# vfrantc/Bayesian-Enhancement-Model

Hardware: AMD Instinct MI355X
Metric: images/sec (whole node) CG_UNet N=8 Bayesian eval @256x256 (higher is better)
Workload: dtype f32

## Files before the change

bayesian-enhancement-model_amd/bem/native.py:

```python
from __future__ import annotations

import ctypes
import os
from ctypes import c_double, c_float, c_int, c_int64, c_uint64, c_void_p

_HERE = os.path.dirname(os.path.abspath(__file__))
LIB_PATH = os.environ.get("BEM_HIP_LIB", os.path.join(os.path.dirname(_HERE), "lib", "libbem_hip.so"))
CSRC = os.path.join(os.path.dirname(_HERE), "csrc")


class BemNativeError(RuntimeError):
    pass


class PwArgs(ctypes.Structure):
    _fields_ = [
        ("x1", c_void_p), ("x2", c_void_p), ("C1", c_int), ("C2", c_int), ("in_mode", c_int),
        ("ln_w", c_void_p), ("ln_b", c_void_p), ("ln_eps", c_float),
        ("Wp", c_void_p), ("w_bstride", c_int64),
        ("bias", c_void_p), ("bias_bstride", c_int64),
        ("res", c_void_p),
        ("prelu", c_void_p), ("act", c_int),
        ("out", c_void_p), ("out_mode", c_int), ("Win", c_int),
        ("B", c_int), ("M", c_int), ("K", c_int), ("L", c_int),
# ... 29 lines not shown
    "bem_pack_pw_weight_f32": [P, P, I, I, I, P],
    "bem_pw_packed_elems": [I, I],
    "bem_pw_gemm_x6_f32": [ctypes.POINTER(PwArgs), P],
    "bem_pack_pw_weight_x6": [P, P, I, I, I, P],
    "bem_pack_pw_weight_x6_strided": [P, P, I, I, I, I64, I64, I64, P],
    "bem_pack_pw_weight_x6_jobs": [P, P, I, P, P],
    "bem_pw_x6_packed_elems": [I, I],
    "bem_bnn_sample_pack_x6": [P, P, P, P, I, I, I, U64, U64, P, I, P],
    "bem_store_words": [P, P, I, P],
    "bem_bnn_ebank_sample_f32": [P, P, I, P, U64, U64, P],
    "bem_bnn_bank_sample_f32": [P, P, I, P, P, P, P, P, F, P, U64, U64, P, P],
    "bem_bnn_bank_kl_f32": [P, P, I, P, P, P, P],
    "bem_bnn_bank_kl_bwd_f32": [P, P, I, P, P, P, P],
    "bem_bnn_bank_reparam_bwd_f32": [P, P, I, P, P, P],
    "bem_row_scale_f32": [P, P, P, I, I, P],
    "bem_se_gate_f32": [P, P, P, P, I, I, I, P],
    "bem_spatial_attention_f32": [P, P, P, P, P, I, I, I, I, I, P],
    "bem_hamilton_bwd_f32": [P, P, P, I, I, I, P],
    "bem_chan_scale_f32": [P, P, I64, P, P, F, P, I, I, I64, P],
    "bem_chan_dot_f32": [P, P, P, I, I, I64, I, P],
    "bem_se_gate_bwd_f32": [P, P, P, P, P, P, P, P, I, I, I, P],
    "bem_spatial_attention_bwd_f32": [P, P, P, P, P, P, P, I, I, I, I, I, P],
    "bem_bnn_prior_ema_f32": [P, P, P, P, F, P, I64, P],
    "bem_bnn_kl_f32": [P, P, P, P, I64, P, P],
    "bem_bnn_kl_bwd_f32": [P, P, P, P, I64, P, P, P, P],
    "bem_bnn_reparam_bwd_f32": [P, P, P, P, P, I64, P],
    "bem_mask_token_f32": [P, P, P, P, I, I, I, I, P],
    "bem_mask_token_bwd_f32": [P, P, P, P, I, I, I, I, P],
    "bem_depth_to_space_f32": [P, P, I, I, I, I, P],
    "bem_prelu_f32": [P, P, P, I64, P],
    "bem_prelu_bwd_f32": [P, P, P, P, P, I64, P],
    "bem_bilinear_up_bwd_f32": [P, P, I, I, I, I, I, P],
    "bem_gdmlp_x6_f32": [P, P, P, F, P, P, P, P, P, P, I, I, I, I, I, P],
    "bem_conv3x3_x6_f32": [P, I64, P, P, P, P, P, I, I, I, I, I, I, P],
    "bem_conv4x4s2_x6_f32": [P, I64, P, P, P, P, P, I, I, I, I, I, I, P],
    "bem_conv4x4s2_fast_supported": [I, I, I],
    "bem_conv3x3_rows_supported": [I, I, I],
    "bem_ss2d_front_x6_f32": [P, P, P, F, P, P, P, P, P, P, P, I, I, I, I, I, P],
    "bem_conv_taps_x6_f32": [P, I64, P, P, P, P, P, I, I, I, I, I, I, I, I, I, P],
    "bem_dwconv3x3_f32": [P, P, I64, P, I64, P, I, I, I, I, I, P],
    "bem_conv2d_f32": [P, I64, P, P, P, P, P, I, I, I, I, I, I, I, I, I, I, P],
    "bem_conv2d_mfma_f32": [P, I64, P, P, P, P, P, I, I, I, I, I, I, I, I, I, I, P],
    "bem_quat_dwt_f32": [P, I64, P, I, I, I, P],
    "bem_dwt_f32": [P, P, I, I, I, I, P],
    "bem_iwt_f32": [P, P, I, I, I, I, P],
    "bem_iwt_hamilton_f32": [P, P, P, I, I, I, P],
    "bem_hamilton_f32": [P, P, I, I, I, P],
    "bem_hamilton_full_f32": [P, P, P, I, I, I, P],
    "bem_attn_stats_f64": [P, P, P, I, I, P],
    "bem_attn_fold_f32": [P, P, P, P, P, P, I, I, P],
    "bem_transpose_planes_f32": [P, I64, P, I64, I, I, I, I, P],
    "bem_copy_channels_f32": [P, I64, P, I64, I, I, I, P],
    "bem_copy_channels_rep_f32": [P, I64, P, I64, I, I, I, I, P],
    "bem_add_channels_f32": [P, I64, P, I64, I, I, I, P],
    "bem_bilinear_up_f32": [P, I64, P, I64, I, I, I, I, I, P],
    "bem_space_to_depth_f32": [P, P, I, I, I, I, P],
    "bem_pixel_shuffle2_f32": [P, P, I, I, I, I, P],
    "bem_bnn_sample_f32": [P, P, P, P, I, I64, U64, U64, P, P],
    "bem_select_best_f32": [P, P, P, P, P, I, I, I64, P],
    "bem_ssim_f32": [P, P, P, P, I, I, I, I, P],
    "bem_select_scores_f32": [P, P, P, F, I, P, P, P, P, I, I, I64, P],
    "bem_mc_mean_f32": [P, P, P, P, I, I, I, I, I, I, I, P],
    "bem_pad_reflect_f32": [P, P, I, I, I, I, I, P],
    "bem_resize_down_f32": [P, P, I, I, I, I, P],
    "bem_randn_f32": [P, I64, U64, U64, P, P],
    "bem_cond_postproc_f32": [P, P, P, P, I, I, I, I, F, P],
# ... 57 lines not shown
```

bayesian-enhancement-model_amd/bem/ops.py:

```python
from __future__ import annotations

import ctypes
import os
from typing import Optional

import torch

from . import native
from .native import PwArgs, check, lib


def _stream():
    return ctypes.c_void_p(torch.cuda.current_stream().cuda_stream)


def _p(t: Optional[torch.Tensor]):
    return ctypes.c_void_p(0 if t is None else t.data_ptr())


def _chk(t: Optional[torch.Tensor], name: str, dtype=torch.float32, optional=False):
    if t is None:
        if optional:
            return
        raise ValueError(f"{name} is required")
# ... 246 lines not shown
    if ln_w.numel() != C or ln_b.numel() != C or dww.numel() != 9 * C or (dwb is not None and dwb.numel() != C) or (bias_in is not None and bias_in.numel() != C):
        raise ValueError("ss2d_front: parameter shapes")
    for Wp, (M, K), nm in ((Wp_in, (C, C), "Wp_in"), (Wp_x, (Mx, C), "Wp_x")):
        if Wp.dim() != 2 or Wp.shape[0] != 1 or Wp.shape[1] != packed_elems(M, K, True) or getattr(Wp, "_bem_mk", (M, K)) != (M, K):
            raise ValueError(f"ss2d_front: {nm} {tuple(Wp.shape)} does not match M={M} K={K} (x6 format, one weight set)")
    xc = torch.empty_like(x)
    xd = torch.empty(B, Mx, H, W, device=x.device, dtype=x.dtype)
    check(lib().bem_ss2d_front_x6_f32(_p(x), _p(ln_w), _p(ln_b), float(ln_eps), _p(Wp_in), _p(bias_in), _p(dww), _p(dwb), _p(Wp_x), _p(xc), _p(xd),
                                      B, C, Mx, H, W, _stream()), "ss2d_front")
    return xc, xd


def gate_interleave(Hd, device):
    j = torch.arange(Hd // 16, device=device)[:, None, None]
    c = torch.arange(16, device=device)[None, :, None]
    s_ = torch.arange(2, device=device)[None, None, :]
    return (s_ * Hd + 16 * j + c).reshape(-1)


GDMLP_X6 = os.environ.get("BEM_GDMLP_X6", "1") != "0"
GDMLP_X6_MAXC = int(os.environ.get("BEM_GDMLP_X6_MAXC", "80"))


def gdmlp_x6_supported(C, Hd):
    return USE_X6 and GDMLP_X6 and C <= GDMLP_X6_MAXC and Hd % 16 == 0


def dw_gate_params10(dww, dwb, Hd):
    w = dww.reshape(2, Hd, 9).permute(1, 2, 0)
    b = torch.zeros(Hd, 1, 2, device=dww.device, dtype=dww.dtype) if dwb is None else dwb.reshape(2, Hd).t().reshape(Hd, 1, 2)
    return torch.cat([w, b], 1).contiguous()


def gdmlp_x6(x, ln_w, ln_b, ln_eps, Wp_gate, bias_gate, dw10, Wp_out, bias_out, Hd):
    for n_, t in (("x", x), ("ln_w", ln_w), ("ln_b", ln_b), ("Wp_gate", Wp_gate), ("bias_gate", bias_gate), ("dw10", dw10), ("Wp_out", Wp_out)):
        _chk(t, n_)
    _chk(bias_out, "bias_out", optional=True)
    B, C, H, W = x.shape
    if not (USE_X6 and C <= 80 and Hd % 16 == 0):
        raise ValueError(f"gdmlp_x6: C = {C} (<= 80) / Hd = {Hd} (% 16) not supported")
    if tuple(dw10.shape) != (Hd, 10, 2):
        raise ValueError("gdmlp_x6: depthwise parameters must come from dw_gate_params10")
    if ln_w.numel() != C or ln_b.numel() != C or bias_gate.numel() != 2 * Hd or (bias_out is not None and bias_out.numel() != C):
        raise ValueError("gdmlp_x6: parameter shapes")
    for Wp, (M, K), nm in ((Wp_gate, (2 * Hd, C), "Wp_gate"), (Wp_out, (C, Hd), "Wp_out")):
        if Wp.dim() != 2 or Wp.shape[0] != 1 or Wp.shape[1] != packed_elems(M, K, True) or getattr(Wp, "_bem_mk", (M, K)) != (M, K):
            raise ValueError(f"gdmlp_x6: {nm} {tuple(Wp.shape)} does not match M={M} K={K} (x6 format, one weight set)")
    out = torch.empty_like(x)
    s = _timed("gdmlp_x6", 8.0 * x.numel(), 6.0 * 2.0 * B * H * W * (2 * Hd * C + Hd * C)) if _PROF is not None and _PROF["kernel"] == "gdmlp_x6" and _PROF["pred"](C) else None
    check(lib().bem_gdmlp_x6_f32(_p(x), _p(ln_w), _p(ln_b), float(ln_eps), _p(Wp_gate), _p(bias_gate), _p(dw10), _p(Wp_out),
                                 _p(bias_out), _p(out), B, C, Hd, H, W, _stream()), "gdmlp_x6")
    _timed_end(s)
    return out


def dwconv3x3(x, w, bias=None, mode=0):
    _chk(x, "x"); _chk(w, "w"); _chk(bias, "bias", optional=True)
    B, Cin, H, W = x.shape
    Cout = Cin // 2 if mode == 2 else Cin
    per_b = w.dim() == 5
    Cw = w.shape[1] if per_b else w.shape[0]
    if Cw != Cin or tuple(w.shape[-3:]) != (1, 3, 3) or (per_b and w.shape[0] != B):
        raise ValueError(f"dwconv3x3: weight {tuple(w.shape)} vs input channels {Cin}")
    bb = 0
    if bias is not None:
        if bias.shape[-1] != Cin:
# ... 961 lines not shown
```

bayesian-enhancement-model_amd/csrc/gdmlp_x6.hip:

```cpp
#include "bem_common.h"
#include "x6_common.h"

namespace {

struct GdX {
    const float* x; const float* ln_w; const float* ln_b; float ln_eps;
    const u32x4* Wpi;
    const u32x4* Wpo;
    const float* bgi;
    const float* dw10;
    int C, Hd, H, W, NCH, tx;
};

constexpr int GD_TH = 4, GD_TW = 32, GD_HW = GD_TW + 2;
constexpr int GD_NPH = (GD_TH + 2) * GD_HW;
constexpr int GD_NPB = (GD_NPH + 31) / 32;
constexpr int GD_TS = 208;
constexpr int GD_GS = 20;

typedef float f32x4 __attribute__((ext_vector_type(4)));

__device__ __forceinline__ float gelu_gate1(float a, float b) {
    const float t = __builtin_amdgcn_rcpf(fmaf(0.3275911f * 0.70710678118654752440f, fabsf(a), 1.f));
    float p = fmaf(1.061405429f, t, -1.453152027f);
    p = fmaf(p, t, 1.421413741f);
    p = fmaf(p, t, -0.284496736f);
    p = fmaf(p, t, 0.254829592f);
    const float e = __builtin_amdgcn_exp2f(a * a * -0.72134752044448170368f);
    const float r = fmaf(-(p * t), e, 1.f);
    const float h = 0.5f * a;
    return fmaf(h, copysignf(r, a), h) * b;
}

template <int KBM, int MTO, int WOB, bool PL2>
__global__ __launch_bounds__(256, 2) void gdmlp_x6_kernel(GdX k, const float* __restrict__ bpo, float bomul, float* __restrict__ out) {
    constexpr int NPI = 3 * KBM, NPO = 3 * MTO;
    __shared__ __attribute__((aligned(16))) f32x2 T[16 * GD_TS];
    __shared__ __attribute__((aligned(16))) float G[128 * GD_GS];
    __shared__ __attribute__((aligned(16))) u32x4 Wis[2][NPI * 64];
    __shared__ __attribute__((aligned(16))) u32x4 Wos[WOB][NPO * 64];
    __shared__ __attribute__((aligned(16))) f32x2 Bss[2][16];
    __shared__ __attribute__((aligned(16))) f32x2 DWs[2][16 * 10];
    const int lane = threadIdx.x & 63, wave = __builtin_amdgcn_readfirstlane(threadIdx.x >> 6), kh = lane >> 5, n = lane & 31;
    const int b = blockIdx.z;
    const int tile = xcd_tile(blockIdx.x, gridDim.x);
    const int tyi = tile / k.tx, txi = tile - tyi * k.tx;
    const int y0 = tyi * GD_TH, x0 = txi * GD_TW;
    const int L = k.H * k.W;
    const float* xb = k.x + (int64_t)b * k.C * L;

    const uint32_t voff = 16 * lane;
    const uint32_t wi_lds = lds_addr(Wis), wo_lds = lds_addr(Wos), bs_lds = lds_addr(Bss), dw_lds = lds_addr(DWs);
    auto dma_in = [&](int ji, int buf) {
#pragma unroll
        for (int t = 0; t < (NPI + 3) / 4; ++t) {
            const int p = wave + 4 * t;
            if (p < NPI) glds16(k.Wpi + ((int64_t)ji * NPI + p) * 64, voff, wi_lds + (buf * NPI + p) * 1024);
        }
        if (wave == (NPI & 3)) {
            const float* src = k.dw10 + (int64_t)ji * 320;
            glds16(src, voff, dw_lds + buf * 1280);
            if (lane < 16) glds16(src + 256, voff, dw_lds + buf * 1280 + 1024);
        }
        if (wave == ((NPI + 1) & 3) && lane < 8) glds16(k.bgi + (int64_t)ji * 32, voff, bs_lds + buf * 128);
    };
    auto dma_out = [&](int jo, int buf) {
#pragma unroll
        for (int t = 0; t < (NPO + 3) / 4; ++t) {
            const int p = wave + 4 * t, mt = p / 3, li = p - 3 * mt;
            if (p < NPO) glds16(k.Wpo + (((int64_t)mt * k.NCH + jo) * 3 + li) * 64, voff, wo_lds + (buf * NPO + p) * 1024);
        }
    };
    dma_in(0, 0);

    const int oy = y0 + wave, ox = x0 + n;
    f32x16 rs[MTO];
    const bool opix = oy < k.H && ox < k.W;
    const int64_t po = (int64_t)min(oy, k.H - 1) * k.W + min(ox, k.W - 1);
    auto load_res = [&]() {
        const float* rb = xb + po;
#pragma unroll
        for (int mt = 0; mt < MTO; ++mt)
#pragma unroll
            for (int r = 0; r < 16; ++r) {
                const int row = min(32 * mt + (r & 3) + 8 * (r >> 2) + 4 * kh, k.C - 1);
                rs[mt][r] = fmaf(bpo[row], bomul, rb[(int64_t)row * L]);
            }
    };

    u32x4 xl[2][KBM][3];
    float msk[2];
    uint32_t mbit[2];
    int hpo[2];
    {
        float lnw[KBM][8], lnb[KBM][8];
#pragma unroll
        for (int kb = 0; kb < KBM; ++kb)
#pragma unroll
            for (int e = 0; e < 8; ++e) {
                const int ch = 16 * kb + 8 * kh + e;
                const float on = ch < k.C ? 1.f : 0.f;
                lnw[kb][e] = k.ln_w[min(ch, k.C - 1)] * on;
                lnb[kb][e] = k.ln_b[min(ch, k.C - 1)] * on;
            }
        float xr[2][KBM][8];
        auto load_block = [&](int i) {
            const int hp = min((wave + 4 * i) * 32 + n, GD_TS - 1);
            hpo[i] = hp;
            const int hy = hp / GD_HW, hx = hp - hy * GD_HW;
            const int gy = y0 - 1 + hy, gx = x0 - 1 + hx;
            const bool in = hp < GD_NPH && gy >= 0 && gy < k.H && gx >= 0 && gx < k.W && (wave + 4 * i) < GD_NPB;
            msk[i] = in ? 1.f : 0.f;
            mbit[i] = in ? 0xffffffffu : 0u;
            const int off = min(max(gy, 0), k.H - 1) * k.W + min(max(gx, 0), k.W - 1);
#pragma unroll
            for (int kb = 0; kb < KBM; ++kb)
#pragma unroll
                for (int e = 0; e < 8; ++e) {
                    const int ch = 16 * kb + 8 * kh + e;
                    const float v = xb[(int64_t)min(ch, k.C - 1) * L + off];
                    xr[i][kb][e] = ch < k.C ? v : 0.f;
                }
        };
        auto norm_block = [&](int i) {
            const float inv = 1.f / (float)k.C;
            float s = 0.f;
#pragma unroll
            for (int kb = 0; kb < KBM; ++kb)
#pragma unroll
                for (int e = 0; e < 8; ++e) s += xr[i][kb][e];
            s += __shfl_xor(s, 32, 64);
            const float mean = s * inv;
            float q = 0.f;
#pragma unroll
            for (int kb = 0; kb < KBM; ++kb)
#pragma unroll
                for (int e = 0; e < 8; ++e) {
                    const float d = (16 * kb + 8 * kh + e < k.C) ? xr[i][kb][e] - mean : 0.f;
                    q = fmaf(d, d, q);
                }
            q += __shfl_xor(q, 32, 64);
            const float rstd = msk[i] / sqrtf(q * inv + k.ln_eps);
#pragma unroll
            for (int kb = 0; kb < KBM; ++kb) {
                float v[8];
#pragma unroll
                for (int e = 0; e < 8; ++e) v[e] = ((xr[i][kb][e] - mean) * rstd) * lnw[kb][e] + lnb[kb][e] * msk[i];
                split8(v, xl[i][kb][0], xl[i][kb][1], xl[i][kb][2]);
            }
        };
        if (PL2) { load_block(0); load_block(1); norm_block(0); norm_block(1); }
        else { load_block(0); norm_block(0); load_block(1); norm_block(1); }
    }

    const int wb_lds = 2 * kh * GD_HW + n;
    const int c_lo = 4 * wave;

    f32x16 oh[MTO];
#pragma unroll
    for (int mt = 0; mt < MTO; ++mt)
#pragma unroll
        for (int r = 0; r < 16; ++r) oh[mt][r] = 0.f;

    auto phase_c = [&](const u32x4* Wo) {
        const float* gp = G + (wave * 32 + n) * GD_GS + 8 * kh;
        const f32x4 ga = *reinterpret_cast<const f32x4*>(gp), gb = *reinterpret_cast<const f32x4*>(gp + 4);
        const float v[8] = {ga[0], ga[1], ga[2], ga[3], gb[0], gb[1], gb[2], gb[3]};
        u32x4 gl[3];
        split8(v, gl[0], gl[1], gl[2]);
#pragma unroll
        for (int mt = 0; mt < MTO; ++mt) {
            const u32x4* wp = Wo + mt * 192 + lane;
            const u32x4 wl[3] = {wp[0], wp[64], wp[128]};
            f32x16 lo;
#pragma unroll
            for (int r = 0; r < 16; ++r) lo[r] = 0.f;
            mac6(wl, gl, oh[mt], lo);
            oh[mt] += lo;
        }
    };

    asm volatile("s_waitcnt vmcnt(0)" ::: "memory");
    __syncthreads();

#pragma clang loop unroll(disable)
    for (int j = 0; j < k.NCH; ++j) {
        const int cur = j & 1;
        if (j + 1 < k.NCH) dma_in(j + 1, cur ^ 1);
        if (WOB == 2) dma_out(j, cur);
        const u32x4* const Wi = Wis[cur];
#pragma unroll
        for (int i = 0; i < 2; ++i) {
            if (wave + 4 * i < GD_NPB) {
                f32x16 hi, lo;
#pragma unroll
                for (int q = 0; q < 8; ++q) {
                    const f32x2 bp = Bss[cur][(q & 1) + 4 * (q >> 1) + 2 * kh];
                    lo[2 * q] = bitsf(fbits(bp[0]) & mbit[i]);
                    lo[2 * q + 1] = bitsf(fbits(bp[1]) & mbit[i]);
                    hi[2 * q] = hi[2 * q + 1] = 0.f;
                }
#pragma unroll
                for (int kb = 0; kb < KBM; ++kb) {
                    const u32x4* wp = Wi + kb * 192 + lane;
                    const u32x4 wl[3] = {wp[0], wp[64], wp[128]};
                    hi = mfma16(wl[0], xl[i][kb][0], hi);
                    lo = mfma16(wl[0], xl[i][kb][2], lo);
                    lo = mfma16(wl[2], xl[i][kb][0], lo);
                    lo = mfma16(wl[1], xl[i][kb][1], lo);
                    lo = mfma16(wl[0], xl[i][kb][1], lo);
                    lo = mfma16(wl[1], xl[i][kb][0], lo);
                }
                f32x2* tp = T + 2 * kh * GD_TS + hpo[i];
#pragma unroll
                for (int q = 0; q < 8; ++q)
                    tp[((q & 1) + 4 * (q >> 1)) * GD_TS] = f32x2{hi[2 * q] + lo[2 * q], hi[2 * q + 1] + lo[2 * q + 1]};
            }
        }
        if (j) phase_c(Wos[(j - 1) & (WOB - 1)]);
        __syncthreads();
        if (WOB == 1) dma_out(j, 0);
        {
            f32x2 g[4];
#pragma unroll
            for (int cc = 0; cc < 4; ++cc) {
                const f32x4* wv = reinterpret_cast<const f32x4*>(DWs[cur] + (c_lo + cc) * 10);
                const f32x4 w01 = wv[0], w23 = wv[1], w45 = wv[2], w67 = wv[3], w8b = wv[4];
                const f32x2 wq[9] = {{w01[0], w01[1]}, {w01[2], w01[3]}, {w23[0], w23[1]}, {w23[2], w23[3]}, {w45[0], w45[1]},
                                     {w45[2], w45[3]}, {w67[0], w67[1]}, {w67[2], w67[3]}, {w8b[0], w8b[1]}};
                const f32x2 bias = {w8b[2], w8b[3]};
                const f32x2* tp = T + (c_lo + cc) * GD_TS + wb_lds;
                f32x2 win[4][3];
#pragma unroll
                for (int dy = 0; dy < 4; ++dy)
#pragma unroll
                    for (int dx = 0; dx < 3; ++dx) win[dy][dx] = tp[dy * GD_HW + dx];
                float a0x = bias[0], a0y = bias[1], a1x = bias[0], a1y = bias[1];
#pragma unroll
                for (int ty = 0; ty < 3; ++ty)
#pragma unroll
                    for (int tx = 0; tx < 3; ++tx) {
                        const f32x2 w = wq[3 * ty + tx], u0 = win[ty][tx], u1 = win[ty + 1][tx];
                        a0x = fmaf(w[0], u0[0], a0x); a0y = fmaf(w[1], u0[1], a0y);
                        a1x = fmaf(w[0], u1[0], a1x); a1y = fmaf(w[1], u1[1], a1y);
                    }
                g[cc] = f32x2{gelu_gate1(a0x, a0y), gelu_gate1(a1x, a1y)};
            }
#pragma unroll
            for (int p = 0; p < 2; ++p)
                *reinterpret_cast<f32x4*>(G + ((2 * kh + p) * 32 + n) * GD_GS + c_lo) = f32x4{g[0][p], g[1][p], g[2][p], g[3][p]};
        }
        asm volatile("s_waitcnt vmcnt(0)" ::: "memory");
        __syncthreads();
    }
    load_res();
    phase_c(Wos[(k.NCH - 1) & (WOB - 1)]);

    if (opix) {
        float* ob = out + (int64_t)b * k.C * L + po;
#pragma unroll
        for (int mt = 0; mt < MTO; ++mt)
#pragma unroll
            for (int r = 0; r < 16; ++r) {
                const int row = 32 * mt + (r & 3) + 8 * (r >> 2) + 4 * kh;
                if (row < k.C) ob[(int64_t)row * L] = oh[mt][r] + rs[mt][r];
            }
    }
}

}

extern "C" int bem_gdmlp_x6_f32(const float* x, const float* ln_w, const float* ln_b, float ln_eps, const float* Wp_gate,
                                const float* bias_gate, const float* dw_gate10, const float* Wp_out,
                                const float* bias_out, float* out, int B, int C, int Hd, int H, int W, void* stream) {
    BEM_REQUIRE(x && ln_w && ln_b && Wp_gate && bias_gate && dw_gate10 && Wp_out && out, "gdmlp_x6: null tensor");
    BEM_REQUIRE(B >= 0 && B <= 65535 && C > 0 && C <= 80 && Hd > 0 && Hd % 16 == 0 && H > 0 && W > 0,
                "gdmlp_x6: needs C <= 80 and Hd %% 16 == 0 (got C = %d, Hd = %d)", C, Hd);
    BEM_REQUIRE((((uintptr_t)Wp_gate | (uintptr_t)Wp_out | (uintptr_t)bias_gate | (uintptr_t)dw_gate10) & 15) == 0,
                "gdmlp_x6: packed weights, bias pairs and depthwise parameters must be 16-byte aligned");
    BEM_REQUIRE(x != out, "gdmlp_x6: in-place operation is not supported (halo reads)");
    BEM_REQUIRE((int64_t)C * H * W < (1ll << 31), "gdmlp_x6: plane set too large for 32-bit offsets");
    if (B == 0) return BEM_OK;
    GdX k;
    k.x = x; k.ln_w = ln_w; k.ln_b = ln_b; k.ln_eps = ln_eps;
    k.Wpi = reinterpret_cast<const u32x4*>(Wp_gate); k.Wpo = reinterpret_cast<const u32x4*>(Wp_out); k.bgi = bias_gate;
    k.dw10 = dw_gate10;
    k.C = C; k.Hd = Hd; k.H = H; k.W = W; k.NCH = Hd / 16; k.tx = cdiv(W, GD_TW);
    const float* bpop = bias_out ? bias_out : ln_w;
    const float bomul = bias_out ? 1.f : 0.f;
    dim3 grid(k.tx * cdiv(H, GD_TH), 1, B);
    hipStream_t s = (hipStream_t)stream;
    const int KB = cdiv(C, 16);
    if (KB == 1) gdmlp_x6_kernel<1, 1, 2, false><<<grid, 256, 0, s>>>(k, bpop, bomul, out);
    else if (KB == 2) gdmlp_x6_kernel<2, 1, 2, false><<<grid, 256, 0, s>>>(k, bpop, bomul, out);
    else if (KB == 3) gdmlp_x6_kernel<3, 2, 2, false><<<grid, 256, 0, s>>>(k, bpop, bomul, out);
    else if (KB == 4) gdmlp_x6_kernel<4, 2, 2, false><<<grid, 256, 0, s>>>(k, bpop, bomul, out);
    else gdmlp_x6_kernel<5, 3, 1, false><<<grid, 256, 0, s>>>(k, bpop, bomul, out);
    return bem_check_launch("gdmlp_x6");
}
```

include/bem_hip.h:

```cpp
#ifndef BEM_HIP_H
#define BEM_HIP_H

#include <stdint.h>

#ifdef __cplusplus
extern "C" {
#endif

#define BEM_OK 0
#define BEM_ERR_INVALID 1
#define BEM_ERR_LAUNCH 2

const char* bem_last_error(void);
int bem_abi_version(void);


int bem_selective_scan_fwd_f32(const float* u, const float* delta, const float* A, const float* Bm,
                               const float* Cm, const float* D, const float* delta_bias, float* out,
                               int batch, int dim, int L, int dstate, int ngroups, int delta_softplus,
                               void* stream);

int bem_selective_scan_fwd_in16(const void* u, const void* delta, const float* A, const void* Bm, const void* Cm, const float* D,
                                const float* delta_bias, float* out, int in_dtype, int batch, int dim, int L, int dstate,
                                int ngroups, int delta_softplus, void* stream);
// ... 102 lines not shown
                              int k, void* stream);

int bem_chan_scale_f32(const float* x, const float* scale, int64_t scale_bstride, const float* add, const float* add_bc, float add_bc_scale,
                       float* out, int B, int C, int64_t HW, void* stream);
int bem_chan_dot_f32(const float* a, const float* b, float* out, int B, int C, int64_t HW, int per_batch, void* stream);
int bem_se_gate_bwd_f32(const float* mean, const float* w1, const float* w2, const float* y, const float* dy, float* dmean, float* dw1,
                        float* dw2, int B, int C, int Cr, void* stream);
int bem_spatial_attention_bwd_f32(const float* x, const float* dout, const float* map, const float* w, float* dpre_ws, float* dx, float* dw,
                                  int B, int C, int H, int W, int k, void* stream);

int bem_bnn_sample_f32(const float* mu, const float* rho, const float* eps_in, float* out,
                       int nsets, int64_t n, uint64_t seed, uint64_t stream_id, const uint64_t* stream_add, void* stream);
int bem_pad_reflect_f32(const float* x, float* out, int P, int H, int W, int Hp, int Wp, void* stream);
int bem_resize_down_f32(const float* x, float* out, int P, int Hp, int Wp, int s, void* stream);
int bem_randn_f32(float* out, int64_t n, uint64_t seed, uint64_t stream_id, const uint64_t* stream_add, void* stream);
int bem_cond_postproc_f32(const float* pred, const float* target_mean, const float* noise, float* out,
                          int Bn, int h, int w, int samples_per_image, float noise_level, void* stream);
int bem_plane_mean_f32(const float* x, float* means, int P, int Hs, int Ws, int h, int w, void* stream);
int bem_candidate_finalize_f32(const float* pred, const float* target, float* final_out, float* psnr, double* ws,
                               int Bn, int samples_per_image, int Hp, int Wp, int h, int w, int gt_mean,
                               void* stream);

int bem_select_best_f32(const float* cand, const float* psnr, int* best, float* best_psnr, float* best_img, int B, int N,
                        int64_t chw, void* stream);

int bem_ssim_f32(const float* pred, const float* target, float* ssim, double* ws, int Bn, int samples_per_image, int h, int w, void* stream);

int bem_select_scores_f32(const float* cand, const float* s1, const float* s2, float weight, int rule, int* best, float* best_s1,
                          float* best_s2, float* best_img, int B, int N, int64_t chw, void* stream);

int bem_mc_mean_f32(const float* pred, const float* target, float* out, double* ws, int B, int N, int Hp, int Wp, int h, int w,
                    int gt_mean, void* stream);

int bem_gdmlp_x6_f32(const float* x, const float* ln_w, const float* ln_b, float ln_eps, const float* Wp_gate,
                     const float* bias_gate, const float* dw_gate10, const float* Wp_out,
                     const float* bias_out, float* out, int B, int C, int Hd, int H, int W, void* stream);

int bem_ss2d_front_x6_f32(const float* x, const float* ln_w, const float* ln_b, float ln_eps, const float* Wp_in, const float* bias_in,
                          const float* dww, const float* dwb, const float* Wp_x, float* xc, float* xd, int B, int C, int Mx, int H, int W,
                          void* stream);


int bem_l1_loss_f32(const float* pred, const float* gt, float* dpred, float* loss, double* ws, int64_t n, float weight,
                    const float* gmul, void* stream);

int bem_iwt_hamilton_bwd_f32(const float* q1w, const float* q2w, const float* dout, float* dq1w, float* dq2w, int B, int h, int w,
                             void* stream);
int bem_hamilton_bwd_f32(const float* q8, const float* dout, float* dq8, int B, int H, int W, void* stream);

int bem_pixel_unshuffle2_f32(const float* x, float* out, int B, int C, int H, int W, void* stream);

int bem_channel_sum_f32(const float* x, float* out, int B, int C, int64_t L, void* stream);
int bem_add_f32(const float* a, const float* b, float* out, int64_t n, float alpha, void* stream);

int bem_ln_bwd_f32(const float* x1, const float* x2, const float* dn, const float* gamma, const float* beta, float eps,
                   const float* dres, float* dx, float* n_out, float* dgamma, float* dbeta, int B, int C, int64_t L, void* stream);
int bem_ln_fwd_f32(const float* x1, const float* x2, const float* gamma, const float* beta, float eps, float* n_out, int B, int C,
                   int64_t L, void* stream);

int bem_dwact_bwd_f32(const float* t, const float* w, const float* bias, const float* dout, float* dpre, float* dw, float* dbias,
                      int B, int Cout, int H, int W, int mode, void* stream);

typedef struct {
    const float* dy; int64_t dy_bstride; int M;
    const float* x1; int64_t x1_bstride; int C1;
    const float* x2; int64_t x2_bstride; int C2;
// ... 55 lines not shown
```

bayesian-enhancement-model_amd/csrc/pw_gemm_x6.hip:

```cpp
#include "bem_common.h"
#include "x6_common.h"
#include <stdlib.h>
#include <algorithm>

namespace {


struct PwX {
    const float* x1; const float* x2; int C1; int C2; int in_mode;
    const float* ln_w; const float* ln_b; float ln_eps;
    const u32x4* Wp; int64_t w_bstride;
    const float* bias; int64_t bias_bstride;
    const float* res; const float* prelu; int act;
    float* out; int out_mode; int Win;
    int M; int K; int L; int KB; int MT;
    int mtpb;
};


template <int NSUB, bool SUM, bool VEC>
__device__ __forceinline__ void ldx(const PwX& k, int b, int ch, int pc, const bool (&keep)[NSUB], float (&o)[NSUB]) {
    const int chc = min(ch, k.K - 1);
    const bool first = chc < k.C1;
    const float* r1 = k.x1 + ((int64_t)b * k.C1 + (first ? chc : 0)) * k.L;
// ... 385 lines not shown
    for (int kb = 0; kb < KBM; ++kb) {
        float v[8];
#pragma unroll
        for (int e = 0; e < 8; ++e) v[e] = xr[kb][e][0];
        split8(v, xl[kb][0], xl[kb][1], xl[kb][2]);
    }
    int buf = 0;
    for (int mt0 = mt_lo; mt0 < mt_hi; ++mt0, buf ^= 1) {
        asm volatile("s_waitcnt vmcnt(0)" ::: "memory");
        __syncthreads();
        if (mt0 + 1 < mt_hi) dma(mt0 + 1, buf ^ 1);
        f32x16 acc[1][1], alo;
        float4 bq[1][4];
        x6_load_bias<1>(k, b, mt0, kh, bq);
#pragma unroll
        for (int r = 0; r < 16; ++r) acc[0][0][r] = alo[r] = 0.f;
        const u32x4* wl = &Ws[buf][lane];
        u32x4 wn[3] = {wl[0], wl[64], wl[128]};
#pragma unroll
        for (int kb = 0; kb < KBM; ++kb) {
            const u32x4 wc[3] = {wn[0], wn[1], wn[2]};
            if (kb + 1 < KBM) {
                wn[0] = wl[((kb + 1) * 3 + 0) * 64]; wn[1] = wl[((kb + 1) * 3 + 1) * 64]; wn[2] = wl[((kb + 1) * 3 + 2) * 64];
            }
            __builtin_amdgcn_sched_barrier(0);
            mac6(wc, xl[kb], acc[0][0], alo);
            __builtin_amdgcn_sched_barrier(0);
        }
        acc[0][0] += alo;
        x6_epilogue<1, 1, VEC>(k, b, mt0, p, keep, kh, s_bias, bq, acc);
    }
}

constexpr int BEM_X6_MAXK_LN = 1024;
template <int MTW, int NSUB, bool SUM, bool VEC, bool LN>
__global__ __launch_bounds__(256, 2) void pw_x6_stream_kernel(PwX k) {
    const int lane = threadIdx.x & 63, wave = threadIdx.x >> 6, kh = lane >> 5, n = lane & 31;
    const int b = blockIdx.z, mt0 = blockIdx.y * MTW;
    const int p0 = (xcd_tile(blockIdx.x, gridDim.x) * 4 + wave) * (32 * NSUB);
    __shared__ __attribute__((aligned(16))) float s_bias[BEM_X6_MAXM];
    __shared__ float s_ln[LN ? 2 * BEM_X6_MAXK_LN : 2];
    stage_bias(k, b, s_bias);
    if (LN) {
        for (int i = threadIdx.x; i < k.KB * 16; i += 256) {
            s_ln[i] = i < k.K ? k.ln_w[i] : 0.f;
            s_ln[BEM_X6_MAXK_LN + i] = i < k.K ? k.ln_b[i] : 0.f;
        }
    }
    __syncthreads();
    if (p0 >= k.L) return;
    const int p = p0 + NSUB * n;
    bool keep[NSUB];
#pragma unroll
    for (int t = 0; t < NSUB; ++t) keep[t] = p + t < k.L;
    const int pc = VEC ? (keep[0] ? p : 0) : p;
    auto load_x = [&](int kb, float (&dst)[8][NSUB]) {
#pragma unroll
        for (int e = 0; e < 8; ++e) ldx<NSUB, SUM, VEC>(k, b, 16 * kb + 8 * kh + e, pc, keep, dst[e]);
    };
    float mean[NSUB], rstd[NSUB];
    if (LN) {
        const float inv = 1.f / (float)k.K;
        float s[NSUB];
#pragma unroll
        for (int t = 0; t < NSUB; ++t) s[t] = 0.f;
        for (int kb = 0; kb < k.KB; ++kb) {
// ... 208 lines not shown
    const int MT = cdiv(M, 32), KB = cdiv(K, 16);
    const int64_t total = (int64_t)nsets * MT * KB * 64;
    sample_pack_x6_kernel<<<(unsigned)cdiv64(total, 256), 256, 0, (hipStream_t)stream>>>(mu, rho, eps_in, reinterpret_cast<u32x4*>(Wp), M, K, MT, KB,
                                                                                       total, seed, stream_id, stream_add, sigma_given);
    return bem_check_launch("bnn_sample_pack_x6");
}

extern "C" int64_t bem_pw_x6_packed_elems(int M, int K) {
    return (int64_t)cdiv(M, 32) * cdiv(K, 16) * 3 * 64 * 4;
}

extern "C" int bem_pack_pw_weight_x6_strided(const float* W, float* Wp, int nsets, int M, int K, int64_t set_stride, int64_t row_stride,
                                             int64_t col_stride, void* stream) {
    BEM_REQUIRE(W && Wp, "pack_pw_weight_x6: null tensor");
    BEM_REQUIRE(nsets >= 0 && M > 0 && K > 0 && set_stride >= 0 && row_stride >= 0 && col_stride >= 0, "pack_pw_weight_x6: bad shape / strides");
    BEM_REQUIRE(((uintptr_t)Wp & 15) == 0, "pack_pw_weight_x6: output must be 16-byte aligned");
    if (nsets == 0) return BEM_OK;
    const int MT = cdiv(M, 32), KB = cdiv(K, 16);
    const int64_t total = (int64_t)nsets * MT * KB * 64;
    pack_x6_kernel<<<(unsigned)cdiv64(total, 256), 256, 0, (hipStream_t)stream>>>(W, reinterpret_cast<u32x4*>(Wp), M, K, MT, KB, total, set_stride,
                                                                                 row_stride, col_stride);
    return bem_check_launch("pack_pw_weight_x6");
}

extern "C" int bem_pack_pw_weight_x6_jobs(const void* jobs, const void* blks, int nblk, float* arena, void* stream) {
    BEM_REQUIRE(jobs && blks && arena && nblk > 0, "pack_pw_weight_x6_jobs: bad arguments");
    BEM_REQUIRE(((uintptr_t)arena & 15) == 0, "pack_pw_weight_x6_jobs: the arena must be 16-byte aligned");
    pack_x6_jobs_kernel<<<nblk, 256, 0, (hipStream_t)stream>>>((const packjob*)jobs, (const int32_t*)blks, arena);
    return bem_check_launch("pack_pw_weight_x6_jobs");
}

extern "C" int bem_pack_pw_weight_x6(const float* W, float* Wp, int nsets, int M, int K, void* stream) {
    return bem_pack_pw_weight_x6_strided(W, Wp, nsets, M, K, (int64_t)M * K, K, 1, stream);
}

extern "C" int bem_pw_gemm_x6_f32(const bem_pw_args* a, void* stream) {
    BEM_REQUIRE(a, "pw_gemm_x6: null args");
    BEM_REQUIRE(a->x1 && a->Wp && a->out, "pw_gemm_x6: null tensor");
    BEM_REQUIRE(a->B >= 0 && a->B <= 65535 && a->M > 0 && a->M <= BEM_X6_MAXM && a->K > 0 && a->L >= 0, "pw_gemm_x6: bad shape B=%d M=%d K=%d L=%d", a->B, a->M, a->K, a->L);
    BEM_REQUIRE(a->in_mode >= 0 && a->in_mode <= 2, "pw_gemm_x6: in_mode %d", a->in_mode);
    if (a->in_mode == 0) BEM_REQUIRE(a->K == a->C1, "pw_gemm_x6: K %d != C1 %d", a->K, a->C1);
    if (a->in_mode == 1) BEM_REQUIRE(a->x2 && a->K == a->C1 && a->C1 == a->C2, "pw_gemm_x6: sum mode needs x2 and K == C1 == C2");
    if (a->in_mode == 2) BEM_REQUIRE(a->x2 && a->K == a->C1 + a->C2, "pw_gemm_x6: cat mode needs x2 and K == C1 + C2");
    BEM_REQUIRE((a->ln_w == nullptr) == (a->ln_b == nullptr), "pw_gemm_x6: ln_w / ln_b must both be set or both NULL");
    BEM_REQUIRE(a->act == 0 || (a->act == 1 && a->prelu), "pw_gemm_x6: act %d", a->act);
    BEM_REQUIRE(a->out_mode == 0 || (a->out_mode == 1 && a->M % 4 == 0 && a->Win > 0 && a->L % a->Win == 0 && !a->res),
                "pw_gemm_x6: out_mode %d constraints", a->out_mode);
    BEM_REQUIRE(((uintptr_t)a->Wp & 15) == 0 && a->w_bstride % 4 == 0, "pw_gemm_x6: packed weights must be 16-byte aligned");
    BEM_REQUIRE((int64_t)a->M * a->L < (1ll << 30), "pw_gemm_x6: M * L = %lld exceeds the 32-bit lane offsets of the epilogue", (long long)a->M * a->L);
    const bool ln = a->ln_w != nullptr;
    BEM_REQUIRE(!ln || a->K <= BEM_X6_MAXK_LN, "pw_gemm_x6: LayerNorm prologue supports K <= %d (got %d)", BEM_X6_MAXK_LN, a->K);
    if (a->B == 0 || a->L == 0) return BEM_OK;
    PwX k;
    k.x1 = a->x1; k.x2 = a->x2 ? a->x2 : a->x1; k.C1 = a->C1; k.C2 = a->x2 ? a->C2 : a->C1; k.in_mode = a->in_mode;
    k.ln_w = a->ln_w; k.ln_b = a->ln_b; k.ln_eps = a->ln_eps;
    k.Wp = reinterpret_cast<const u32x4*>(a->Wp); k.w_bstride = a->w_bstride / 4; k.bias = a->bias; k.bias_bstride = a->bias_bstride;
    k.res = a->res; k.prelu = a->prelu; k.act = a->act; k.out = a->out; k.out_mode = a->out_mode; k.Win = a->Win;
    k.M = a->M; k.K = a->K; k.L = a->L; k.KB = cdiv(a->K, 16); k.MT = cdiv(a->M, 32); k.mtpb = k.MT;
    hipStream_t s = (hipStream_t)stream;
    const bool sum = a->in_mode == 1;
    const bool al = (((uintptr_t)a->x1 | (uintptr_t)(a->x2 ? a->x2 : a->x1) | (uintptr_t)a->out | (uintptr_t)(a->res ? a->res : a->out)) & 7) == 0;
    const bool vec = a->L % 2 == 0 && al;
#define BEM_X6_RES(KBM, NSUB, MTW)                                                                       \
    do {                                                                                                 \
        dim3 grid(cdiv(a->L, 128 * NSUB), 1, a->B);                                                      \
                    \
        const int64_t wv = (int64_t)a->B * cdiv(a->L, 32 * NSUB);                                        \
        const int groups = cdiv(k.MT, MTW);                                                              \
        const int ny = wv >= 2048 ? 1 : (int)std::min<int64_t>(groups, cdiv64(2048, wv));                \
        k.mtpb = cdiv(groups, ny) * MTW;                                                                 \
        grid.y = cdiv(k.MT, k.mtpb);                                                                     \
        if (NSUB == 2 && vec && !sum) pw_x6_res_kernel<KBM, NSUB, MTW, false, true><<<grid, 256, 0, s>>>(k);   \
        else if (NSUB == 2 && vec) pw_x6_res_kernel<KBM, NSUB, MTW, true, true><<<grid, 256, 0, s>>>(k);       \
        else if (!sum) pw_x6_res_kernel<KBM, NSUB, MTW, false, false><<<grid, 256, 0, s>>>(k);                 \
        else pw_x6_res_kernel<KBM, NSUB, MTW, true, false><<<grid, 256, 0, s>>>(k);                            \
        return bem_check_launch("pw_x6_res");                                                            \
    } while (0)
    if (k.KB <= 3) BEM_X6_RES(3, 2, 1);
    if (ln && k.KB <= 5) BEM_X6_RES(5, 2, 1);
    static const bool res10 = !(getenv("BEM_X6_RES10") && atoi(getenv("BEM_X6_RES10")) == 0);
    static const bool reslds = !(getenv("BEM_X6_RES_LDS") && atoi(getenv("BEM_X6_RES_LDS")) == 0);
    if (ln && k.KB == 10 && k.K == 160 && k.MT >= 8 && res10 && reslds && (int64_t)a->B * cdiv(a->L, 32) >= 2048) {
        dim3 grid(cdiv(a->L, 128), 1, a->B);
        k.mtpb = k.MT;
        if (!sum) pw_x6_res_lds_kernel<10, false, false><<<grid, 256, 0, s>>>(k);
        else pw_x6_res_lds_kernel<10, true, false><<<grid, 256, 0, s>>>(k);
        return bem_check_launch("pw_x6_res_lds");
    }
    if (ln && k.KB <= 10 && res10) { if (k.MT == 1) BEM_X6_RES(10, 1, 1); else BEM_X6_RES(10, 1, 2); }
#undef BEM_X6_RES
    {
        const bool three = false && k.MT == 3 && !ln;
        const int mtw = three ? 3 : (k.MT == 1 ? 1 : 2);
        dim3 grid(cdiv(a->L, three ? 128 : 256), cdiv(k.MT, mtw), a->B);
#define BEM_X6_STREAM(MTW, LN)                                                                \
    do {                                                                                      \
// ... 208 lines not shown
```

Before: 319.9.

## Cheaper GELU-gate polynomial, LDS zero-fill for halo masks, split accumulators in gdmlp

Replaces the erf-based GELU approximation in the fused gated MLP kernel with a clamped degree-6 polynomial in exponent form. This removes the reciprocal and leaves one exp2, shortening the per-element gate math. Out-of-image halo pixels are now zeroed once in LDS, which drops the per-use bitmask AND in the inner loop. For small MTO the kernel keeps a persistent second MFMA accumulator instead of zeroing and adding a temporary per step, at the cost of extra registers. A standalone gelu_gate kernel and its binding are also added, likely for testing the new approximation, which may differ slightly in accuracy.

After: 324.6, median of 6. 1.5% higher.

```diff
diff --git a/bayesian-enhancement-model_amd/bem/native.py b/bayesian-enhancement-model_amd/bem/native.py
--- a/bayesian-enhancement-model_amd/bem/native.py
+++ b/bayesian-enhancement-model_amd/bem/native.py
@@ -85,6 +85,7 @@
     "bem_prelu_bwd_f32": [P, P, P, P, P, I64, P],
     "bem_bilinear_up_bwd_f32": [P, P, I, I, I, I, I, P],
     "bem_gdmlp_x6_f32": [P, P, P, F, P, P, P, P, P, P, I, I, I, I, I, P],
+    "bem_gdmlp_gelu_gate_f32": [P, P, P, I64, P],
     "bem_conv3x3_x6_f32": [P, I64, P, P, P, P, P, I, I, I, I, I, I, P],
     "bem_conv4x4s2_x6_f32": [P, I64, P, P, P, P, P, I, I, I, I, I, I, P],
     "bem_conv4x4s2_fast_supported": [I, I, I],
diff --git a/bayesian-enhancement-model_amd/bem/ops.py b/bayesian-enhancement-model_amd/bem/ops.py
--- a/bayesian-enhancement-model_amd/bem/ops.py
+++ b/bayesian-enhancement-model_amd/bem/ops.py
@@ -302,6 +302,15 @@
     return torch.cat([w, b], 1).contiguous()
 
 
+def gdmlp_gelu_gate(a, b):
+    _chk(a, "a"); _chk(b, "b")
+    if a.shape != b.shape:
+        raise ValueError("gdmlp_gelu_gate: shapes differ")
+    out = torch.empty_like(a)
+    check(lib().bem_gdmlp_gelu_gate_f32(_p(a), _p(b), _p(out), a.numel(), _stream()), "gdmlp_gelu_gate")
+    return out
+
+
 def gdmlp_x6(x, ln_w, ln_b, ln_eps, Wp_gate, bias_gate, dw10, Wp_out, bias_out, Hd):
     for n_, t in (("x", x), ("ln_w", ln_w), ("ln_b", ln_b), ("Wp_gate", Wp_gate), ("bias_gate", bias_gate), ("dw10", dw10), ("Wp_out", Wp_out)):
         _chk(t, n_)
diff --git a/bayesian-enhancement-model_amd/csrc/gdmlp_x6.hip b/bayesian-enhancement-model_amd/csrc/gdmlp_x6.hip
--- a/bayesian-enhancement-model_amd/csrc/gdmlp_x6.hip
+++ b/bayesian-enhancement-model_amd/csrc/gdmlp_x6.hip
@@ -21,15 +21,15 @@
 typedef float f32x4 __attribute__((ext_vector_type(4)));
 
 __device__ __forceinline__ float gelu_gate1(float a, float b) {
-    const float t = __builtin_amdgcn_rcpf(fmaf(0.3275911f * 0.70710678118654752440f, fabsf(a), 1.f));
-    float p = fmaf(1.061405429f, t, -1.453152027f);
-    p = fmaf(p, t, 1.421413741f);
-    p = fmaf(p, t, -0.284496736f);
-    p = fmaf(p, t, 0.254829592f);
-    const float e = __builtin_amdgcn_exp2f(a * a * -0.72134752044448170368f);
-    const float r = fmaf(-(p * t), e, 1.f);
-    const float h = 0.5f * a;
-    return fmaf(h, copysignf(r, a), h) * b;
+    const float u = fabsf(a), uc = fminf(u, 5.6f);
+    float q = fmaf(8.857549801e-06f, uc, -5.768916162e-05f);
+    q = fmaf(q, uc, -4.070074065e-04f);
+    q = fmaf(q, uc, 7.363169454e-03f);
+    q = fmaf(q, uc, -5.266664177e-02f);
+    q = fmaf(q, uc, -4.591643214e-01f);
+    q = fmaf(q, uc, -1.151108861e+00f);
+    const float e = __builtin_amdgcn_exp2f(fmaf(u, q, -1.f));
+    return fmaf(-uc, e, fmaxf(a, 0.f)) * b;
 }
 
 template <int KBM, int MTO, int WOB, bool PL2>
@@ -90,7 +90,6 @@
 
     u32x4 xl[2][KBM][3];
     float msk[2];
-    uint32_t mbit[2];
     int hpo[2];
     {
         float lnw[KBM][8], lnb[KBM][8];
@@ -106,12 +105,15 @@
         float xr[2][KBM][8];
         auto load_block = [&](int i) {
             const int hp = min((wave + 4 * i) * 32 + n, GD_TS - 1);
-            hpo[i] = hp;
             const int hy = hp / GD_HW, hx = hp - hy * GD_HW;
             const int gy = y0 - 1 + hy, gx = x0 - 1 + hx;
             const bool in = hp < GD_NPH && gy >= 0 && gy < k.H && gx >= 0 && gx < k.W && (wave + 4 * i) < GD_NPB;
             msk[i] = in ? 1.f : 0.f;
-            mbit[i] = in ? 0xffffffffu : 0u;
+            hpo[i] = in ? hp : GD_TS - 1;
+            if (!in && hp < GD_NPH) {
+#pragma unroll
+                for (int q = 0; q < 8; ++q) T[((q & 1) + 4 * (q >> 1) + 2 * kh) * GD_TS + hp] = f32x2{0.f, 0.f};
+            }
             const int off = min(max(gy, 0), k.H - 1) * k.W + min(max(gx, 0), k.W - 1);
 #pragma unroll
             for (int kb = 0; kb < KBM; ++kb)
@@ -156,11 +158,16 @@
     const int wb_lds = 2 * kh * GD_HW + n;
     const int c_lo = 4 * wave;
 
-    f32x16 oh[MTO];
+    constexpr bool OLK = MTO <= 2;
+    f32x16 oh[MTO], ol[OLK ? MTO : 1];
 #pragma unroll
     for (int mt = 0; mt < MTO; ++mt)
 #pragma unroll
         for (int r = 0; r < 16; ++r) oh[mt][r] = 0.f;
+#pragma unroll
+    for (int mt = 0; mt < (OLK ? MTO : 1); ++mt)
+#pragma unroll
+        for (int r = 0; r < 16; ++r) ol[mt][r] = 0.f;
 
     auto phase_c = [&](const u32x4* Wo) {
         const float* gp = G + (wave * 32 + n) * GD_GS + 8 * kh;
@@ -172,11 +179,15 @@
         for (int mt = 0; mt < MTO; ++mt) {
             const u32x4* wp = Wo + mt * 192 + lane;
             const u32x4 wl[3] = {wp[0], wp[64], wp[128]};
-            f32x16 lo;
-#pragma unroll
-            for (int r = 0; r < 16; ++r) lo[r] = 0.f;
-            mac6(wl, gl, oh[mt], lo);
-            oh[mt] += lo;
+            if (OLK) {
+                mac6(wl, gl, oh[mt], ol[mt]);
+            } else {
+                f32x16 lo;
+#pragma unroll
+                for (int r = 0; r < 16; ++r) lo[r] = 0.f;
+                mac6(wl, gl, oh[mt], lo);
+                oh[mt] += lo;
+            }
         }
     };
 
@@ -196,8 +207,8 @@
 #pragma unroll
                 for (int q = 0; q < 8; ++q) {
                     const f32x2 bp = Bss[cur][(q & 1) + 4 * (q >> 1) + 2 * kh];
-                    lo[2 * q] = bitsf(fbits(bp[0]) & mbit[i]);
-                    lo[2 * q + 1] = bitsf(fbits(bp[1]) & mbit[i]);
+                    lo[2 * q] = bp[0];
+                    lo[2 * q + 1] = bp[1];
                     hi[2 * q] = hi[2 * q + 1] = 0.f;
                 }
 #pragma unroll
@@ -263,11 +274,23 @@
 #pragma unroll
             for (int r = 0; r < 16; ++r) {
                 const int row = 32 * mt + (r & 3) + 8 * (r >> 2) + 4 * kh;
-                if (row < k.C) ob[(int64_t)row * L] = oh[mt][r] + rs[mt][r];
+                if (row < k.C) ob[(int64_t)row * L] = (OLK ? oh[mt][r] + ol[OLK ? mt : 0][r] : oh[mt][r]) + rs[mt][r];
             }
     }
 }
 
+__global__ void gdmlp_gelu_gate_kernel(const float* __restrict__ a, const float* __restrict__ b, float* __restrict__ out, int64_t n) {
+    const int64_t i = (int64_t)blockIdx.x * blockDim.x + threadIdx.x;
+    if (i < n) out[i] = gelu_gate1(a[i], b[i]);
+}
+
+}
+
+extern "C" int bem_gdmlp_gelu_gate_f32(const float* a, const float* b, float* out, int64_t n, void* stream) {
+    BEM_REQUIRE(a && b && out && n >= 0, "gdmlp_gelu_gate: bad arguments");
+    if (n == 0) return BEM_OK;
+    gdmlp_gelu_gate_kernel<<<(unsigned)cdiv64(n, 256), 256, 0, (hipStream_t)stream>>>(a, b, out, n);
+    return bem_check_launch("gdmlp_gelu_gate");
 }
 
 extern "C" int bem_gdmlp_x6_f32(const float* x, const float* ln_w, const float* ln_b, float ln_eps, const float* Wp_gate,
diff --git a/include/bem_hip.h b/include/bem_hip.h
--- a/include/bem_hip.h
+++ b/include/bem_hip.h
@@ -158,6 +158,7 @@
 int bem_mc_mean_f32(const float* pred, const float* target, float* out, double* ws, int B, int N, int Hp, int Wp, int h, int w,
                     int gt_mean, void* stream);
 
+int bem_gdmlp_gelu_gate_f32(const float* a, const float* b, float* out, int64_t n, void* stream);
 int bem_gdmlp_x6_f32(const float* x, const float* ln_w, const float* ln_b, float ln_eps, const float* Wp_gate,
                      const float* bias_gate, const float* dw_gate10, const float* Wp_out,
                      const float* bias_out, float* out, int B, int C, int Hd, int H, int W, void* stream);
```

## Add persistent software-pipelined pointwise GEMM kernel for small K and M

Applied to the files above, without the earlier changes.

Adds a persistent kernel for pointwise convs with K<=48 and M<=96. It stages all packed weights, bias and LN params into LDS once per block, then has each wave walk over 32-pixel tiles with a grid stride. The next tile's activations are prefetched into registers while the current tile computes, and the first residual tiles are prefetched too. The grid is sized from the CU count to remove per-block setup and hide global load latency, at the cost of higher register pressure and a new dispatch path that is on by default.

Result: no change. 311.7 before, 313.4 after (median of 6 runs) (+0.5%).

```diff
diff --git a/bayesian-enhancement-model_amd/csrc/pw_gemm_x6.hip b/bayesian-enhancement-model_amd/csrc/pw_gemm_x6.hip
--- a/bayesian-enhancement-model_amd/csrc/pw_gemm_x6.hip
+++ b/bayesian-enhancement-model_amd/csrc/pw_gemm_x6.hip
@@ -441,6 +441,161 @@
     }
 }
 
+template <int KBM, int MTN, bool SUM>
+__global__ __launch_bounds__(256, 2) void pw_x6_pipe_kernel(PwX k) {
+    constexpr int NPF = MTN < 2 ? MTN : 2;
+    __shared__ __attribute__((aligned(16))) u32x4 Ws[MTN * KBM * 3 * 64];
+    __shared__ __attribute__((aligned(16))) float s_bias[MTN * 32];
+    __shared__ float s_ln[2 * 16 * KBM];
+    const int lane = threadIdx.x & 63, wave = __builtin_amdgcn_readfirstlane(threadIdx.x >> 6), kh = lane >> 5, n = lane & 31;
+    const int b = blockIdx.z;
+    {
+        const u32x4* wsrc = k.Wp + (int64_t)b * k.w_bstride;
+        const int per = k.KB * 3;
+        for (int piece = wave; piece < MTN * per; piece += 4) {
+            const int mt = piece / per;
+            glds16(wsrc + (int64_t)piece * 64, (uint32_t)lane * 16u, lds_addr(&Ws[(mt * KBM * 3 + piece - mt * per) * 64]));
+        }
+        for (int i = threadIdx.x; i < MTN * KBM * 3 * 64; i += 256)
+            if ((i >> 6) % (KBM * 3) >= per) Ws[i] = u32x4{0u, 0u, 0u, 0u};
+        const float* bias = k.bias ? k.bias + (int64_t)b * k.bias_bstride : nullptr;
+        for (int i = threadIdx.x; i < MTN * 32; i += 256) s_bias[i] = (bias && i < k.M) ? bias[i] : 0.f;
+        for (int i = threadIdx.x; i < 16 * KBM; i += 256) {
+            const bool on = k.ln_w && i < k.K;
+            s_ln[i] = on ? k.ln_w[min(i, k.K - 1)] : 0.f;
+            s_ln[16 * KBM + i] = on ? k.ln_b[min(i, k.K - 1)] : 0.f;
+        }
+        asm volatile("s_waitcnt vmcnt(0)" ::: "memory");
+        __syncthreads();
+    }
+    const int nt = (k.L + 31) >> 5, tstride = gridDim.x * 4;
+    int t = blockIdx.x * 4 + wave;
+    if (t >= nt) return;
+    const float slope = k.act == 1 ? k.prelu[0] : 0.f;
+    const bool act = k.act == 1, cat = k.in_mode == 2, has_res = k.res != nullptr;
+    struct Sh { const float* x1; const float* x2; const float* res; float* out; int L, K, M, C1; };
+    auto shape = [&]() {
+        Sh s{k.x1 + (int64_t)b * k.C1 * k.L, k.x2 + (int64_t)b * k.C2 * k.L, (has_res ? k.res : k.out) + (int64_t)b * k.M * k.L,
+             k.out + (int64_t)b * k.M * k.L, k.L, k.K, k.M, k.C1};
+        asm volatile("" : "+s"(s.x1), "+s"(s.x2), "+s"(s.res), "+s"(s.out), "+s"(s.L), "+s"(s.K), "+s"(s.M), "+s"(s.C1));
+        return s;
+    };
+    float xa[KBM][8], xs[KBM][SUM ? 8 : 1];
+    auto load_tile = [&](const Sh& s, int tt) {
+        const int pc = min(tt * 32 + n, s.L - 1);
+        const uint32_t lo = (uint32_t)(8 * kh) * (uint32_t)s.L + (uint32_t)pc;
+#pragma unroll
+        for (int kb = 0; kb < KBM; ++kb)
+#pragma unroll
+            for (int e = 0; e < 8; ++e) {
+                const int u = 16 * kb + e;
+                float& a = xa[kb][e];
+                float& x2v = xs[kb][SUM ? e : 0];
+                if (u + 8 < s.K && (!cat || u + 8 < s.C1 || u >= s.C1)) {
+                    a = ((cat && u >= s.C1) ? s.x2 + (int64_t)(u - s.C1) * s.L : s.x1 + (int64_t)u * s.L)[lo];
+                    if (SUM) x2v = (s.x2 + (int64_t)u * s.L)[lo];
+                } else {
+                    const int chc = min(u + 8 * kh, s.K - 1);
+                    a = (chc < s.C1 ? s.x1 + (int64_t)chc * s.L : s.x2 + (int64_t)(chc - s.C1) * s.L)[pc];
+                    if (SUM) x2v = (s.x2 + (int64_t)chc * s.L)[pc];
+                }
+            }
+    };
+    load_tile(shape(), t);
+    for (; t < nt; t += tstride) {
+        const Sh s = shape();
+        const int p = t * 32 + n;
+        const bool keep = p < s.L;
+        const int pc = min(p, s.L - 1);
+        const uint32_t loff = (uint32_t)(4 * kh) * (uint32_t)s.L + (uint32_t)pc;
+        auto load_res = [&](int mt, float (&dst)[16]) {
+#pragma unroll
+            for (int r = 0; r < 16; ++r) {
+                const int urow = mt * 32 + 8 * (r >> 2) + (r & 3);
+                dst[r] = (s.res + (int64_t)min(urow, s.M - 1) * s.L)[urow + 4 * kh < s.M ? loff : (uint32_t)pc];
+            }
+        };
+        float rv[NPF > 0 ? NPF : 1][16];
+        if (has_res) {
+#pragma unroll
+            for (int mt = 0; mt < NPF; ++mt) load_res(mt, rv[mt]);
+        }
+        float xr[KBM][8];
+#pragma unroll
+        for (int kb = 0; kb < KBM; ++kb)
+#pragma unroll
+            for (int e = 0; e < 8; ++e) {
+                float v = xa[kb][e];
+                if (SUM) v += xs[kb][e];
+                const float mk = 16 * kb + 8 * kh + e < s.K ? 1.f : 0.f;
+                xr[kb][e] = keep ? v * mk : 0.f;
+            }
+        if (t + tstride < nt) load_tile(s, t + tstride);
+        if (k.ln_w) {
+            const float inv = 1.f / (float)s.K;
+            float sm = 0.f;
+#pragma unroll
+            for (int kb = 0; kb < KBM; ++kb)
+#pragma unroll
+                for (int e = 0; e < 8; ++e) sm += xr[kb][e];
+            sm += __shfl_xor(sm, 32, 64);
+#pragma unroll
+            for (int kb = 0; kb < KBM; ++kb)
+#pragma unroll
+                for (int e = 0; e < 8; ++e) xr[kb][e] = fmaf(-inv, sm, xr[kb][e]);
+            float q = 0.f;
+#pragma unroll
+            for (int kb = 0; kb < KBM; ++kb)
+#pragma unroll
+                for (int e = 0; e < 8; ++e) {
+                    const float d = (16 * kb + 8 * kh + e < s.K) ? xr[kb][e] : 0.f;
+                    q = fmaf(d, d, q);
+                }
+            q += __shfl_xor(q, 32, 64);
+            const float rstd = 1.f / sqrtf(q * inv + k.ln_eps);
+#pragma unroll
+            for (int kb = 0; kb < KBM; ++kb)
+#pragma unroll
+                for (int e = 0; e < 8; ++e) {
+                    const float g = valu_copy(s_ln[16 * kb + 8 * kh + e]), be = valu_copy(s_ln[16 * KBM + 16 * kb + 8 * kh + e]);
+                    xr[kb][e] = xr[kb][e] * rstd * g + be;
+                }
+        }
+        u32x4 xl[KBM][3];
+#pragma unroll
+        for (int kb = 0; kb < KBM; ++kb) split8(xr[kb], xl[kb][0], xl[kb][1], xl[kb][2]);
+#pragma unroll
+        for (int mt = 0; mt < MTN; ++mt) {
+            __builtin_amdgcn_sched_barrier(0);
+            float rl[16];
+            if (mt >= NPF && has_res) load_res(mt, rl);
+            f32x16 acc, alo;
+#pragma unroll
+            for (int r = 0; r < 16; ++r) acc[r] = alo[r] = 0.f;
+            const u32x4* wl = &Ws[mt * KBM * 3 * 64 + lane];
+#pragma unroll
+            for (int kb = 0; kb < KBM; ++kb) {
+                const u32x4 w[3] = {wl[(kb * 3 + 0) * 64], wl[(kb * 3 + 1) * 64], wl[(kb * 3 + 2) * 64]};
+                mac6(w, xl[kb], acc, alo);
+            }
+            acc += alo;
+#pragma unroll
+            for (int g = 0; g < 4; ++g) {
+                const float4 b4 = *reinterpret_cast<const float4*>(&s_bias[mt * 32 + 8 * g + 4 * kh]);
+                const float bv[4] = {valu_copy(b4.x), valu_copy(b4.y), valu_copy(b4.z), valu_copy(b4.w)};
+#pragma unroll
+                for (int i = 0; i < 4; ++i) {
+                    const int r = 4 * g + i, urow = mt * 32 + 8 * g + i;
+                    float o = acc[r] + bv[i];
+                    if (act) o = o >= 0.f ? o : slope * o;
+                    if (has_res) o += mt < NPF ? rv[mt < NPF ? mt : 0][r] : rl[r];
+                    if (keep && urow + 4 * kh < s.M) (s.out + (int64_t)urow * s.L)[loff] = o;
+                }
+            }
+        }
+    }
+}
+
 constexpr int BEM_X6_MAXK_LN = 1024;
 template <int MTW, int NSUB, bool SUM, bool VEC, bool LN>
 __global__ __launch_bounds__(256, 2) void pw_x6_stream_kernel(PwX k) {
@@ -715,6 +870,14 @@
 
 extern "C" int bem_pack_pw_weight_x6(const float* W, float* Wp, int nsets, int M, int K, void* stream) {
     return bem_pack_pw_weight_x6_strided(W, Wp, nsets, M, K, (int64_t)M * K, K, 1, stream);
+}
+
+static int x6_cu_count() {
+    static int ncu[64] = {};
+    int dev = 0;
+    if (hipGetDevice(&dev) != hipSuccess || dev < 0 || dev >= 64) return 0;
+    if (!ncu[dev] && hipDeviceGetAttribute(&ncu[dev], hipDeviceAttributeMultiprocessorCount, dev) != hipSuccess) ncu[dev] = 0;
+    return ncu[dev];
 }
 
 extern "C" int bem_pw_gemm_x6_f32(const bem_pw_args* a, void* stream) {
@@ -744,7 +907,22 @@
     const bool sum = a->in_mode == 1;
     const bool al = (((uintptr_t)a->x1 | (uintptr_t)(a->x2 ? a->x2 : a->x1) | (uintptr_t)a->out | (uintptr_t)(a->res ? a->res : a->out)) & 7) == 0;
     const bool vec = a->L % 2 == 0 && al;
-#define BEM_X6_RES(KBM, NSUB, MTW)                                                                       \
+    static const bool pipe = !(getenv("BEM_X6_PIPE") && atoi(getenv("BEM_X6_PIPE")) == 0);
+    const int ncu = pipe ? x6_cu_count() : 0;
+    if (ncu > 0 && k.KB <= 3 && k.MT <= 3 && a->out_mode == 0 && a->M >= 8 && (int64_t)a->B * cdiv(a->L, 32) >= 8 * 4 * 2 * (int64_t)ncu) {
+        dim3 grid((unsigned)std::max(1, std::min(cdiv(a->L, 128), cdiv(2 * ncu, a->B))), 1, a->B);
+#define BEM_X6_PIPE(KBM, MTN)                                                      \
+    do {                                                                           \
+        if (sum) pw_x6_pipe_kernel<KBM, MTN, true><<<grid, 256, 0, s>>>(k);         \
+        else pw_x6_pipe_kernel<KBM, MTN, false><<<grid, 256, 0, s>>>(k);            \
+    } while (0)
+        if (k.MT == 1) BEM_X6_PIPE(3, 1);
+        else if (k.MT == 2) BEM_X6_PIPE(3, 2);
+        else BEM_X6_PIPE(3, 3);
+#undef BEM_X6_PIPE
+        return bem_check_launch("pw_x6_pipe");
+    }
+#define BEM_X6_RES(KBM, NSUB, MTW)                                                                    \
     do {                                                                                                 \
         dim3 grid(cdiv(a->L, 128 * NSUB), 1, a->B);                                                      \
                     \
```
